# Villen-Lab/pyAscore

Measured on AMD Instinct MI355X. Metric: PSMs/sec (Ascore.score) at 1/2/4/8 MI355X + HBM-roofline %, higher is better.
Workload: dtype f32/f64 scalar + i32 counts

## Files before the change

pyascore_amd/csrc/fused_core.hip.h:

```cpp
#ifndef PYA_FUSED_CORE_H
#define PYA_FUSED_CORE_H
#include "score_core.hip.h"
#include "localize_core.hip.h"

#define FUSED_ROUND 3

struct FusedLds {
    uint16_t *grid;
    uint4 *cum_lut;
    PeakEntry *peaks;
    float2 *resd;
    uint8_t *rkl;
    uint32_t *rec;
    float *wsl;
    float *mass_l;
    uint32_t *flag_l;
    uint8_t *site_pos;
    float *selm;
    unsigned char *sort_raw;
    PushedEntry *pushed;
    unsigned long long *site_alt;
    uint32_t *site_max, *site_tie, *n_pushed;
    float *sc;
    uint32_t *c_tr, *c_cnt;
    uint32_t *bad_tasks;
    uint32_t *t_lo, *t_off;
    float *srt_v;
    uint8_t *srt_h;
    int32_t *c_depth;
    uint32_t *c_site;
};

__host__ __device__ static inline size_t fused_align16(size_t v) { return (v + 15) & ~(size_t)15; }
__host__ __device__ static inline size_t fused_sort_bytes(uint32_t n) {
    if (n <= 64) return ((size_t)n * 10 + 15) & ~(size_t)15;
    return (((size_t)n * 6 + 15) & ~(size_t)15) + ((size_t)n / 64 + 2) * 16 + 2 * 128 * 2;
}
__host__ __device__ static inline uint32_t fused_site_cap(uint32_t push_cap) {
    const uint32_t v = (push_cap + 3u) & ~3u;
    return v > 64u ? 64u : (v < 4u ? 4u : v);
}
__host__ __device__ static inline size_t fused_post_bytes(uint32_t n_cap, uint32_t push_cap, uint32_t ent_cap, uint32_t ndir,
                                                          bool multi_z) {
    return fused_align16(fused_sort_bytes(n_cap)) + (size_t)push_cap * 16 + (size_t)fused_site_cap(push_cap) * 16 + 16 +
           (size_t)(1 + FUSED_ROUND) * 40 + (size_t)FUSED_ROUND * (16 * ndir + 4 + 4) + 16 + 64 +
           (multi_z ? fused_align16((size_t)FUSED_ROUND * ndir * 2 * ent_cap * 4) +
                          fused_align16((size_t)FUSED_ROUND * ndir * 2 * ent_cap)
                    : 0);
}
__host__ __device__ static inline size_t fused_walk_bytes(uint32_t cap) {
    return 16 * 16 + ((size_t)cap + PYA_TABLE_PAD) * 8;
}
__host__ __device__ static inline size_t fused_kept_bytes(uint32_t n_cap, uint32_t stride, uint32_t pos_cap, uint32_t ent_cap,
                                                          uint32_t ndir) {
    return fused_align16(((size_t)pos_cap + 1) * 8) + fused_align16((size_t)ent_cap * stride) + (size_t)n_cap * 16 + 256 +
           fused_align16((size_t)pos_cap + 1) + (size_t)(1 + FUSED_ROUND) * ndir * ent_cap * 4;
}
__host__ __device__ static inline size_t fused_lds_bytes(uint32_t cap, uint32_t n_cap, uint32_t stride, uint32_t pos_cap,
                                                         uint32_t ent_cap, uint32_t push_cap, uint32_t ndir, bool multi_z) {
    const size_t walk = fused_walk_bytes(cap), post = fused_post_bytes(n_cap, push_cap, ent_cap, ndir, multi_z);
    return PYA_GRID_CELLS * 2 + fused_align16(walk > post ? walk : post) +
           fused_kept_bytes(n_cap, stride, pos_cap, ent_cap, ndir) + 16;
}

DEV FusedLds fused_carve(unsigned char *raw, uint32_t cap, uint32_t n_cap, uint32_t stride, uint32_t pos_cap,
                         uint32_t ent_cap, uint32_t push_cap, uint32_t ndir, bool multi_z) {
    FusedLds f;
    f.grid = (uint16_t *)raw;
    size_t o = PYA_GRID_CELLS * 2;
    f.cum_lut = (uint4 *)(raw + o);
    f.peaks = (PeakEntry *)(raw + o + 16 * 16);
    f.sort_raw = raw + o;
    size_t q = o + fused_align16(fused_sort_bytes(n_cap));
    f.pushed = (PushedEntry *)(raw + q);
    q += (size_t)push_cap * sizeof(PushedEntry);
    const size_t sc = fused_site_cap(push_cap);
    f.site_alt = (unsigned long long *)(raw + q);
    q += sc * 8;
    f.site_max = (uint32_t *)(raw + q);
    q += sc * 4;
    f.site_tie = (uint32_t *)(raw + q);
    q += sc * 4;
    f.n_pushed = (uint32_t *)(raw + q);
    q += 16;
    f.sc = (float *)(raw + q);
    q += (size_t)(1 + FUSED_ROUND) * 40;
    f.c_tr = (uint32_t *)(raw + q);
    q += (size_t)FUSED_ROUND * ndir * 8;
    f.c_cnt = (uint32_t *)(raw + q);
    q += (size_t)FUSED_ROUND * ndir * 8;
    f.c_depth = (int32_t *)(raw + q);
    q += FUSED_ROUND * 4;
    f.c_site = (uint32_t *)(raw + q);
    q += FUSED_ROUND * 4;
    f.bad_tasks = (uint32_t *)(raw + q);
    q += 16;
    f.t_lo = (uint32_t *)(raw + q);
    f.t_off = f.t_lo + 8;
    q += 64;
    f.srt_v = (float *)(raw + q);
    q += fused_align16((size_t)FUSED_ROUND * ndir * 2 * ent_cap * 4);
    f.srt_h = (uint8_t *)(raw + q);
    const size_t walk = fused_walk_bytes(cap), post = fused_post_bytes(n_cap, push_cap, ent_cap, ndir, multi_z);
    o += fused_align16(walk > post ? walk : post);
    f.resd = (float2 *)(raw + o);
    o += fused_align16(((size_t)pos_cap + 1) * 8);
    f.rkl = (uint8_t *)(raw + o);
    o += fused_align16((size_t)ent_cap * stride);
    f.rec = (uint32_t *)(raw + o);
    o += (size_t)n_cap * 12;
    f.wsl = (float *)(raw + o);
    o += (size_t)n_cap * 4;
    f.mass_l = (float *)(raw + o);
    f.flag_l = (uint32_t *)(raw + o + 128);
    f.site_pos = (uint8_t *)(raw + o + 256);
    f.selm = (float *)(raw + o + 256 + fused_align16((size_t)pos_cap + 1));
    return f;
}


template <bool BZ>
DEV void walk_record_steps(const float2 *&rp, int rstride, StepBits &bits, float &running, const uint4 *lut, CumCounts &cum,
                           const PeakTable &tab, int zmax, double A, double B, uint8_t *&ro, int stride, int count) {
    for (int i = 0; i < count; i++, rp += rstride) {
        const float2 mm = *rp;
        running = (bits.next() ? mm.y : mm.x) + running;
        const double m = BZ ? (double)running + A : ((double)running + A) - B;
        for (int z = 1; z <= zmax; z++, ro += stride) {
            const Look k = look4(tab, charge_mz(m, z));
            int rk = k.best;
            if (k.more()) rk = look_rest(tab, k);
            cum.add(lut[rk]);
            *ro = (uint8_t)rk;
        }
    }
}
DEV CumCounts walk_record(const float2 *resd, const uint4 *lut, const PeakTable &tab, int L, int zmax, uint64_t resmask, int dir,
                          double A, double B, bool all_b_zero, uint8_t *rkl, int stride, int w) {
    const uint64_t tmask = dir ? (__brevll(resmask) >> (64 - L)) : resmask;
    const float2 *rp = resd + (dir ? L - 1 : 0);
    const int rstride = dir ? -1 : 1;
    uint8_t *ro = rkl + w;
    float running = 0.f;
    CumCounts cum = {0u, 0u, 0u};
    if (tab.half_check) {
        const uint32_t tlo = (uint32_t)tmask, thi = (uint32_t)(tmask >> 32);
        for (int step = 0; step + 1 < L; step++, rp += rstride) {
            const float2 mm = *rp;
            const uint32_t word = step < 32 ? tlo : thi;
            const bool mod = (word >> (step & 31)) & 1u;
            running = (mod ? mm.y : mm.x) + running;
            const double m = ((double)running + A) - B;
            for (int z = 1; z <= zmax; z++, ro += stride) {
                const int rk = match_rank_lds(tab, charge_mz(m, z));
                cum.add(lut[rk]);
                *ro = (uint8_t)rk;
            }
        }
        return cum;
    }
    const uint64_t M = msb_first_from(tmask, 0);
    const int n = L - 1;
    for (int seg = 0; seg < 2; seg++) {
        StepBits bits = {seg ? (uint32_t)M : (uint32_t)(M >> 32)};
        int c = (n < seg * 32 + 32 ? n : seg * 32 + 32) - seg * 32;
        if (c < 0) c = 0;
        if (all_b_zero) walk_record_steps<true>(rp, rstride, bits, running, lut, cum, tab, zmax, A, B, ro, stride, c);
        else walk_record_steps<false>(rp, rstride, bits, running, lut, cum, tab, zmax, A, B, ro, stride, c);
    }
    return cum;
}

DEV void walk_mz_only(const float2 *resd, int L, int zmax, uint64_t resmask, int dir, double A, double B, float *out) {
    const uint64_t tmask = dir ? (__brevll(resmask) >> (64 - L)) : resmask;
    const uint64_t M = msb_first_from(tmask, 0);
    const float2 *rp = resd + (dir ? L - 1 : 0);
    const int rstride = dir ? -1 : 1;
    const int Lm1 = L - 1;
    float running = 0.f;
    int step = 0;
    for (int seg = 0; seg < 2; seg++) {
        StepBits bits = {seg ? (uint32_t)M : (uint32_t)(M >> 32)};
        const int end = Lm1 < seg * 32 + 32 ? Lm1 : seg * 32 + 32;
        for (; step < end; step++, rp += rstride) {
            const float2 mm = *rp;
            running = (bits.next() ? mm.y : mm.x) + running;
            const double m = ((double)running + A) - B;
            out[step] = (float)(m + 1.007825);
            for (int z = 2; z <= zmax; z++) out[(z - 1) * Lm1 + step] = charge_mz(m, z);
        }
    }
}

DEV void walk_sums_only(const float2 *resd, int L, uint64_t resmask, int dir, float *out) {
    const uint64_t tmask = dir ? (__brevll(resmask) >> (64 - L)) : resmask;
    const uint64_t M = msb_first_from(tmask, 0);
    const float2 *rp = resd + (dir ? L - 1 : 0);
    const int rstride = dir ? -1 : 1;
    const int Lm1 = L - 1;
    float running = 0.f;
    int step = 0;
    for (int seg = 0; seg < 2; seg++) {
        StepBits bits = {seg ? (uint32_t)M : (uint32_t)(M >> 32)};
        const int end = Lm1 < seg * 32 + 32 ? Lm1 : seg * 32 + 32;
        for (; step < end; step++, rp += rstride) {
            const float2 mm = *rp;
            running = (bits.next() ? mm.y : mm.x) + running;
            out[step] = running;
        }
    }
}

DEV int partners_in_run(const float *run, int n, int p2, float me, int side, float err) {
    int j = 0;
    for (int step = p2 >> 1; step > 0; step >>= 1) {
        const int probe = j + step;
        const float o = probe - 1 < n ? run[probe - 1] : __builtin_huge_valf();
        const float dd = side ? (o - me) : (me - o);
        if (side ? (dd <= -err) : (dd >= err)) j = probe;
    }
    int cnt = 0;
    for (int q = j; q < j + 2 && q < n; q++) {
        const float dd = side ? (run[q] - me) : (me - run[q]);
        cnt += (__builtin_fabsf(dd) < err) ? 1 : 0;
    }
    return cnt;
}

#define FUSED_LOCAL_CHUNKS 8
struct LocalTable {
    const float *mz;
    const uint8_t *rank;
    int R, status;
};

template <bool BOTH, bool ZM, bool WIDE = false>
DEV bool fused_body(const BatchDev &b, uint32_t psm, unsigned char *lds_raw, uint32_t cap, uint32_t n_cap, uint32_t stride,
                    uint32_t pos_cap, uint32_t ent_cap, uint32_t push_cap, const LocalTable *local = nullptr) {
    const int lane = lane_id();
    const DevConfig *cfg = b.cfg;
    const int ndir = BOTH ? 2 : 1;
    const FusedLds f = fused_carve(lds_raw, cap, n_cap, stride, pos_cap, ent_cap, push_cap, (uint32_t)ndir, ZM);
    STAMP_BEGIN();
    STAMP_T(b, 38, false);
    float lmz[FUSED_LOCAL_CHUNKS];
    uint32_t lrk[FUSED_LOCAL_CHUNKS];
    if (local) {
#pragma unroll
        for (int q = 0; q < FUSED_LOCAL_CHUNKS; q++) {
            const int i = q * 64 + lane_id();
            lmz[q] = i < local->R ? local->mz[i] : __builtin_huge_valf();
            lrk[q] = i < local->R ? (uint32_t)local->rank[i] : (uint32_t)PYA_NO_MATCH;
        }
        wave_lds_sync();
    }
    if (lane < 32) {
        f.mass_l[lane] = cfg->res_mass[lane];
        f.flag_l[lane] = cfg->res_modifiable[lane];
    }
    const uint64_t *dw = b.desc + (size_t)psm * PYA_DESC_WORDS;
    const int64_t p0 = (int64_t)dw[0], pep0 = (int64_t)dw[1], s0 = (int64_t)dw[2], a0 = (int64_t)dw[3];
    const uint64_t w4 = dw[4], w5 = dw[5];
    const int L = (int)(w4 & 0xffffu), n_aux = (int)((w4 >> 16) & 0xffffu), k = (int)((w4 >> 32) & 0xffffu);
    const int zmax = ZM ? (int)(w4 >> 56) : 1;
    const int N = (int)(uint32_t)w5;
    const uint64_t *order = b.order_tab + (uint32_t)(w5 >> 32);
    const int status = local ? local->status : b.status[psm];
    const int R = local ? local->R : (int)b.ret_n[psm];

    const uint32_t max_k = b.max_k;
    float *out_asc = b.ascores + (size_t)psm * max_k;
    uint64_t *out_alt = b.alt_mask + (size_t)psm * max_k;
    for (uint32_t a = lane; a < max_k; a += 64) {
        out_asc[a] = 0.f;
        out_alt[a] = 0ull;
    }
    if (status != PYA_ST_OK) {
        if (lane == 0) {
            b.best_score[psm] = -1.f;
            b.best_sig[psm] = 0ull;
            b.n_sig_out[psm] = -1;
        }
        return false;
    }
    STAMP_T(b, 39, false);
    const bool two_pass = BOTH && WIDE && N > 32;
    const int s = (BOTH && !two_pass) ? (lane & 31) : lane;
    const int dir = BOTH ? (two_pass ? 0 : (lane >> 5)) : (cfg->n_fwd > 0 ? 0 : 1);
    const bool active = s < N;
    const uint32_t letter = lane < L ? (uint32_t)b.pep[pep0 + lane] : (uint32_t)'A';
    const uint64_t bits = active ? order[s] : 0ull;
    uint32_t aux_pos = 0;
    float aux_mass = 0.f;
    if (lane < n_aux) {
        aux_pos = b.aux_pos[a0 + lane];
        aux_mass = b.aux_mass[a0 + lane];
    }
    if (local) {
#pragma unroll
        for (int q = 0; q < FUSED_LOCAL_CHUNKS; q++) {
            const int i = q * 64 + lane;
            if (i < R + PYA_TABLE_PAD) {
                PeakEntry e;
                e.mz = lmz[q];
                e.rank = lrk[q];
                f.peaks[i] = e;
            }
        }
    } else {
        copy_peak_table(b.ret + p0, R, f.peaks, lane, 64);
    }
    PeakTable tab;
    tab.e = f.peaks;
    tab.g_cell = nullptr;
    tab.g_e = b.ret + p0;
    tab.n = R;
    tab.err = cfg->mz_error;
    tab.half_check = cfg->mz_error > 0.49f;
    double Af = 0., Bf = 0., Ab = 0., Bb = 0.;
    if (cfg->n_fwd > 0) type_constants(cfg->types[0], &Af, &Bf);
    if (cfg->n_fwd < cfg->n_types) type_constants(cfg->types[cfg->n_fwd], &Ab, &Bb);
    wave_lds_sync();
    STAMP_T(b, 48, false);
    float m0, m1;
    uint64_t site_mask;
    {
        const bool in = lane < L;
        const uint32_t li = (letter - 'A') & 31u;
        m0 = f.mass_l[li];
        const bool modifiable = in && ((f.flag_l[li] & 1u) || (cfg->allow_n && lane == 0) || (cfg->allow_c && lane == L - 1));
        m1 = m0 + cfg->mod_mass;
        for (int base = 0; base < n_aux; base += 64) {
            const int n = n_aux - base < 64 ? n_aux - base : 64;
            if (base > 0) {
                aux_pos = 0;
                aux_mass = 0.f;
                if (lane < n) {
                    aux_pos = b.aux_pos[a0 + base + lane];
                    aux_mass = b.aux_mass[a0 + base + lane];
                }
            }
            for (int j = 0; j < n; j++) {
                const uint32_t pos = (uint32_t)__builtin_amdgcn_readlane((int)aux_pos, j);
                const float am = __int_as_float(__builtin_amdgcn_readlane(__float_as_int(aux_mass), j));
                const int idx = pos > 0 ? (int)pos - 1 : 0;
                if (idx == lane) {
                    m0 += am;
                    m1 += am;
                }
            }
        }
        site_mask = __ballot(modifiable);
        if (in) f.resd[lane] = make_float2(m0, m1);
        if (modifiable) f.site_pos[mask_rank(site_mask)] = (uint8_t)lane;
    }
    STAMP_T(b, 49, false);
    grid_build(&tab, f.grid);
    STAMP_T(b, 50, false);
    if (lane < 16) f.cum_lut[lane] = fused_cum_entry((uint32_t)lane);
    const int Lm1 = L - 1;
    const uint64_t resmask = deposit_sites(bits, site_mask);
    const int w = !active ? (int)stride - 1 : (BOTH ? dir * N + s : s);
    const bool presorted = !__any(lane < L && !(m0 > 0.f && m1 > 0.f));
    const float wide_min = 2.f * cfg->mz_error + 0.02f;
    const bool wide = !__any(lane < L && !(m0 > wide_min && m1 > wide_min));
    wave_lds_sync();
    STAMP_T(b, 40, false);
    CumCounts cum = walk_record(f.resd, f.cum_lut, tab, L, zmax, resmask, dir, dir ? Ab : Af, dir ? Bb : Bf, Bf == 0. && Bb == 0.,
                                f.rkl, (int)stride, w);
    if (two_pass) {
        const CumCounts back = walk_record(f.resd, f.cum_lut, tab, L, zmax, resmask, 1, Ab, Bb, Bf == 0. && Bb == 0., f.rkl, (int)stride,
                                           active ? N + s : (int)stride - 1);
        cum.a += back.a;
        cum.b += back.b;
        cum.c += back.c;
    } else if (BOTH) {
        uint32_t *r3 = f.rec + (size_t)s * 3;
        if (active && lane >= 32) {
            r3[0] = cum.a;
            r3[1] = cum.b;
            r3[2] = cum.c;
        }
        wave_lds_sync();
        if (active && lane < 32) {
            cum.a += r3[0];
            cum.b += r3[1];
            cum.c += r3[2];
        }
    }
    wave_lds_sync();
    STAMP_T(b, 41, false);

    const uint32_t nfrag = (uint32_t)ndir * (uint32_t)Lm1 * (uint32_t)zmax;
    int fail = 0;
    float ws = 0.f;
    if (active && (!BOTH || two_pass || lane < 32)) {
        ws = -1.f;
        if (nfrag <= b.lut_n_max) {
            double sum = 0.;
#pragma unroll
            for (int d = 0; d < PYA_NTOP; d++) {
                const float sc = lut_score(b, (uint32_t)d, cum.at(d), nfrag);
                const float prod = cfg->weights[d] * sc;
                sum = sum + (double)prod;
            }
            ws = (float)sum;
        } else {
            fail = 1;
        }
        uint32_t *r3 = f.rec + (size_t)s * 3;
        r3[0] = cum.a;
        r3[1] = cum.b;
        r3[2] = cum.c;
        f.wsl[s] = ws;
    }
    if (__any(fail)) {
        if (lane == 0) {
            b.status[psm] = PYA_ST_LUT_RANGE;
            b.best_score[psm] = -1.f;
            b.best_sig[psm] = 0ull;
            b.n_sig_out[psm] = -1;
        }
        return false;
    }
    wave_lds_sync();
    STAMP_T(b, 42, false);

    bool declined = !presorted || (b.debug & 512);
    const bool sig_lane = lane < N;
    const uint64_t my_bits = bits;
    const float my_ws = sig_lane ? f.wsl[lane] : 0.f;
    float best_ws = 0.f;
    uint64_t best_bits = 0ull;
    uint32_t best_i = 0, np = 0;
    if (!declined) {
        const uint32_t u = sig_lane ? __float_as_uint(my_ws) : 0u;
        const uint32_t kmax = wave_max_u32(u);
        const uint64_t at_max = __ballot(sig_lane && u == kmax);
        best_i = (uint32_t)__builtin_ctzll(at_max);
        if (lane == 0) *f.n_pushed = 0;
        if ((uint32_t)lane < fused_site_cap(push_cap)) {
            f.site_max[lane] = 0;
            f.site_tie[lane] = 0;
            f.site_alt[lane] = 0ull;
        }
        if (__popcll(at_max) != 1 || (b.debug & 1024)) {
            const SortLds srt = sort_carve(f.sort_raw, N);
            if (sig_lane) {
                srt.key[lane] = my_ws;
                srt.idx[lane] = (uint16_t)lane;
            }
            wave_lds_sync();
            if (!(b.debug & 8) && sort_introsort_loop<true, true>(srt, N, true)) declined = true;
            const uint64_t m2 = __ballot(sig_lane && __float_as_uint(srt.key[lane]) == kmax);
            best_i = srt.idx[__builtin_ctzll(m2)];
        }
        best_ws = __uint_as_float(kmax);
        best_bits = __shfl(my_bits, (int)best_i, 64);
        wave_lds_sync();
    }
    STAMP_T(b, 43, false);
    if (!declined) {
        const uint64_t gone = best_bits & ~my_bits, came = my_bits & ~best_bits;
        const bool single = sig_lane && __popcll(gone) == 1 && __popcll(came) == 1;
        const int a = single ? __popcll(best_bits & (gone - 1)) : 0;
        const uint32_t u = __float_as_uint(my_ws);
        if (single) atomicMax(&f.site_max[a], u);
        wave_lds_sync();
        if (single && u == f.site_max[a]) {
            if ((double)__builtin_fabsf(best_ws - my_ws) < 1e-6) {
                f.site_tie[a] = 1u;
                atomicOr(&f.site_alt[a], 1ull << f.site_pos[__builtin_ctzll(came)]);
            } else {
                const uint32_t slot = atomicAdd(f.n_pushed, 1u);
                if (slot < push_cap) {
                    PushedEntry pe;
                    pe.bits = my_bits;
                    pe.ws = my_ws;
                    pe.idx = (uint32_t)lane;
                    f.pushed[slot] = pe;
                }
            }
        }
        wave_lds_sync();
        np = *f.n_pushed;
        if (np > push_cap) np = push_cap;
        if (b.debug & 16) np = 0;
    }
    STAMP_T(b, 44, false);
    float my_asc = __builtin_huge_valf();
    const float err = cfg->mz_error;
    const FastDiv divL = fastdiv_make((uint32_t)(Lm1 > 0 ? Lm1 : 1));
    int p2 = 1;
    while (p2 <= Lm1) p2 <<= 1;
    for (uint32_t e0 = 0; !declined && e0 < np; e0 += FUSED_ROUND) {
        const int nc = (int)(np - e0) < FUSED_ROUND ? (int)(np - e0) : FUSED_ROUND;
        const int S = 1 + nc;
        if (lane < S * ndir && (e0 == 0 || lane >= ndir)) {
            const int sg = lane / ndir, d = lane - sg * ndir;
            const uint64_t sb = sg == 0 ? best_bits : f.pushed[e0 + sg - 1].bits;
            const int dd = BOTH ? d : (cfg->n_fwd > 0 ? 0 : 1);
            if (ZM) walk_mz_only(f.resd, L, zmax, deposit_sites(sb, site_mask), dd, dd ? Ab : Af, dd ? Bb : Bf,
                                 f.selm + (size_t)lane * ent_cap);
            else walk_sums_only(f.resd, L, deposit_sites(sb, site_mask), dd, f.selm + (size_t)lane * ent_cap);
        }
        if (!ZM) {
            wave_lds_sync();
            const int l0 = e0 == 0 ? 0 : ndir, nl = S * ndir - l0;
            for (int i = lane; i < nl * Lm1; i += 64) {
                const int lq = (int)fastdiv((uint32_t)i, divL), st = i - lq * Lm1;
                const int dd = BOTH ? ((l0 + lq) & 1) : (cfg->n_fwd > 0 ? 0 : 1);
                float *at = f.selm + (size_t)(l0 + lq) * ent_cap + st;
                const double m = ((double)*at + (dd ? Ab : Af)) - (dd ? Bb : Bf);
                *at = (float)(m + 1.007825);
            }
        }
        for (int i = (e0 == 0 ? 0 : 10) + lane; i < S * 10; i += 64) {
            const int sg = i / 10, d = i - sg * 10;
            const uint32_t who = sg == 0 ? best_i : f.pushed[e0 + sg - 1].idx;
            const uint32_t cum = (f.rec[(size_t)who * 3 + (d >> 2)] >> ((d & 3) * 8)) & 0xffu;
            f.sc[i] = b.lut[lut_row(nfrag) + (uint32_t)d * (nfrag + 1) + cum];
        }
        wave_lds_sync();
        if (lane < nc) {
            const PushedEntry pe = f.pushed[e0 + lane];
            const uint64_t gone = best_bits & ~pe.bits, came = pe.bits & ~best_bits;
            const int a = __popcll(best_bits & (gone - 1));
            atomicOr(&f.site_alt[a], 1ull << f.site_pos[__builtin_ctzll(came)]);
            f.c_site[lane] = (uint32_t)a;
        }
        {
            const int c = lane >> 4, d = lane & 15;
            const bool on = c < nc && d < PYA_NTOP;
            uint32_t key = 0;
            if (on) {
                const float diff = f.sc[d] - f.sc[(c + 1) * 10 + d];
                key = diff > 0.f ? __float_as_uint(diff) : 0u;
            }
            if (lane < nc) f.c_depth[lane] = 0;
            wave_lds_sync();
            if (on && key) atomicMax((uint32_t *)&f.c_depth[c], key);
            wave_lds_sync();
            const uint64_t at_max = __ballot(on && key && key == (uint32_t)f.c_depth[c]);
            wave_lds_sync();
            if (lane < nc) {
                const uint32_t m16 = (uint32_t)(at_max >> (16 * lane)) & 0xffffu;
                f.c_depth[lane] = m16 ? __builtin_ctz(m16) : 0;
            }
        }
        if (lane < nc * ndir * 2) {
            f.c_tr[lane] = 0;
            f.c_cnt[lane] = 0;
        }
        if (lane == 0) *f.bad_tasks = 0u;
        wave_lds_sync();
        STAMP_T(b, 45, false);
        const int ents = Lm1 * zmax;
        const int items_all = nc * ndir * 2 * ents;
        const FastDiv divE = fastdiv_make((uint32_t)(ents > 0 ? ents : 1));
        const bool spans = !ZM && wide && !(b.debug & 2048);
        const bool zm_clusters = ZM && !(b.debug & 2048);
        int items = items_all;
        if (spans) {
            const int ntask = nc * ndir;
            if (lane < ntask) {
                const int c = lane / ndir, d = lane - c * ndir;
                const int dd = BOTH ? d : (cfg->n_fwd > 0 ? 0 : 1);
                const uint64_t diff = best_bits ^ f.pushed[e0 + c].bits;
                const int r_lo = (int)f.site_pos[__builtin_ctzll(diff)];
                const int r_hi = (int)f.site_pos[63 - __builtin_clzll(diff)];
                const int lo = dd ? L - 1 - r_hi : r_lo, hi = dd ? L - 1 - r_lo : r_hi;
                f.t_lo[lane] = (uint32_t)lo;
                f.t_off[lane] = (uint32_t)(2 * (hi - lo));
            }
            wave_lds_sync();
            uint32_t acc = 0;
            for (int t = 0; t < ntask; t++) {
                const uint32_t n = f.t_off[t];
                wave_lds_sync();
                if (lane == 0) f.t_off[t] = acc;
                acc += n;
            }
            if (lane == 0) f.t_off[ntask] = acc;
            items = (int)acc;
            wave_lds_sync();
        }
        if (!(b.debug & 1) && !zm_clusters)
        for (int base = 0; base < items; base += 64) {
            const int e = base + lane;
            if (e < items) {
                int task, side, en;
                if (spans) {
                    const int ntask = nc * ndir;
                    task = 0;
                    for (int t = 1; t < ntask; t++) task += (uint32_t)e >= f.t_off[t] ? 1 : 0;
                    const int rem = e - (int)f.t_off[task];
                    const int len = (int)(f.t_off[task + 1] - f.t_off[task]) >> 1;
                    side = rem >= len ? 1 : 0;
                    en = (int)f.t_lo[task] + rem - side * len;
                } else {
                    const uint32_t ts = fastdiv((uint32_t)e, divE);
                    en = e - (int)ts * ents;
                    side = (int)ts & 1;
                    task = (int)ts >> 1;
                }
                const int z0 = zmax == 1 ? 0 : (int)fastdiv((uint32_t)en, divL), i = en - z0 * Lm1;
                const int d = BOTH ? task & 1 : 0;
                const int c = BOTH ? task >> 1 : task;
                const float *la = f.selm + (size_t)d * ent_cap;
                const float *lb = f.selm + (size_t)((1 + c) * ndir + d) * ent_cap;
                const float *mine = side ? lb : la, *others = side ? la : lb;
                const float me = mine[en];
                int total = 0;
                {
                    const float *other = others + z0 * Lm1;
                    float df[4];
                    bool ok[4], sk[4];
#pragma unroll
                    for (int uu = 0; uu < 4; uu++) {
                        const int q = i - 1 + uu;
                        ok[uu] = q >= 0 && q < Lm1;
                        const float o = ok[uu] ? other[q] : (q < 0 ? -__builtin_huge_valf() : __builtin_huge_valf());
                        df[uu] = me - o;
                        sk[uu] = df[uu] >= err;
                    }
                    const int w1 = (ok[1] && __builtin_fabsf(df[1]) < err) ? 1 : 0;
                    const int w2 = (ok[2] && __builtin_fabsf(df[2]) < err) ? 1 : 0;
                    const int w3 = (ok[3] && __builtin_fabsf(df[3]) < err) ? 1 : 0;
                    int cnt = -1;
                    if (sk[0] && !sk[1]) cnt = w1 + w2;
                    else if (sk[1] && !sk[2]) cnt = w2 + w3;
                    if (cnt < 0) cnt = partners_in_run(other, Lm1, p2, me, side, err);
                    total = cnt;
                }
                for (int zz = 0; zz < zmax; zz++)
                    if (zz != z0) total += partners_in_run(others + zz * Lm1, Lm1, p2, me, side, err);
                if (total > 1 || (b.debug & 2048)) {
                    atomicOr(f.bad_tasks, 1u << task);
                } else if (total == 0) {
                    const uint32_t who = side ? f.pushed[e0 + c].idx : best_i;
                    atomicAdd(&f.c_tr[task * 2 + side], 1u);
                    if ((int)f.rkl[(size_t)(i * zmax + z0) * stride + (d * N + (int)who)] <= f.c_depth[c])
                        atomicAdd(&f.c_cnt[task * 2 + side], 1u);
                }
            }
        }
        wave_lds_sync();
        const uint32_t bad = zm_clusters ? (1u << (nc * ndir)) - 1u : *f.bad_tasks;
        if (!ZM && bad) declined = true;
        if (ZM && bad && !(b.debug & 1)) {
            for (int base = 0; base < items_all; base += 64) {
                const int e = base + lane;
                if (e < items_all) {
                    const uint32_t ts = fastdiv((uint32_t)e, divE);
                    const int en = e - (int)ts * ents;
                    const int z0 = zmax == 1 ? 0 : (int)fastdiv((uint32_t)en, divL), i = en - z0 * Lm1;
                    const int side = (int)ts & 1;
                    const int d = BOTH ? ((int)ts >> 1) & 1 : 0;
                    const int c = BOTH ? (int)ts >> 2 : (int)ts >> 1;
                    const int task = c * ndir + d;
                    if ((bad >> task) & 1u) {
                        const float *mine = f.selm + (size_t)((side ? (1 + c) * ndir : 0) + d) * ent_cap;
                        const float me = mine[en];
                        int pos = i;
                        for (int zz = 0; zz < zmax; zz++) {
                            if (zz == z0) continue;
                            const float *run = mine + zz * Lm1;
                            int j = 0;
                            for (int step = p2 >> 1; step > 0; step >>= 1) {
                                const int probe = j + step;
                                if (probe - 1 < Lm1 && (zz < z0 ? run[probe - 1] <= me : run[probe - 1] < me)) j = probe;
                            }
                            pos += j;
                        }
                        const uint32_t who = side ? f.pushed[e0 + c].idx : best_i;
                        const size_t at = (size_t)(task * 2 + side) * ent_cap + pos;
                        f.srt_v[at] = me;
                        f.srt_h[at] = (int)f.rkl[(size_t)(i * zmax + z0) * stride + (d * N + (int)who)] <= f.c_depth[c] ? 1 : 0;
                    }
                }
            }
            wave_lds_sync();
            if (zm_clusters) {
                int p2e = 1;
                while (p2e <= ents) p2e <<= 1;
                for (int base = 0; base < items_all; base += 64) {
                    const int e = base + lane;
                    if (e >= items_all) continue;
                    const uint32_t ts = fastdiv((uint32_t)e, divE);
                    const int i = e - (int)ts * ents;
                    const int side = (int)ts & 1;
                    const int d = BOTH ? ((int)ts >> 1) & 1 : 0;
                    const int c = BOTH ? (int)ts >> 2 : (int)ts >> 1;
                    const int task = c * ndir + d;
                    const float *va = f.srt_v + (size_t)(task * 2) * ent_cap, *vb = va + ent_cap;
                    const uint8_t *ha = f.srt_h + (size_t)(task * 2) * ent_cap, *hb = ha + ent_cap;
                    const float *mine = side ? vb : va, *other = side ? va : vb;
                    const float me = mine[i];
                    int j = 0;
                    for (int step = p2e >> 1; step > 0; step >>= 1) {
                        const int probe = j + step;
                        if (probe - 1 < ents && (side ? other[probe - 1] <= me : other[probe - 1] < me)) j = probe;
                    }
                    const float before_own = i > 0 ? mine[i - 1] : -__builtin_huge_valf();
                    const float before_other = j > 0 ? other[j - 1] : -__builtin_huge_valf();
                    if (!(me - before_own >= err && me - before_other >= err)) continue;
                    int ia = side ? j : i, ib = side ? i : j;
                    uint32_t tr0 = 0, tr1 = 0, n0 = 0, n1 = 0;
                    float reached = -__builtin_huge_valf();
                    for (bool first = true;; first = false) {
                        const float xa = ia < ents ? va[ia] : __builtin_huge_valf();
                        const float xb = ib < ents ? vb[ib] : __builtin_huge_valf();
                        const float next = xa <= xb ? xa : xb;
                        if (next == __builtin_huge_valf()) break;
                        if (!first && next - reached >= err) break;
                        if (__builtin_fabsf(xa - xb) < err) {
                            ia++;
                            ib++;
                            reached = __builtin_fmaxf(reached, xa > xb ? xa : xb);
                        } else if (xa < xb) {
                            tr0++;
                            n0 += ha[ia++];
                            reached = __builtin_fmaxf(reached, xa);
                        } else {
                            tr1++;
                            n1 += hb[ib++];
                            reached = __builtin_fmaxf(reached, xb);
                        }
                    }
                    if (tr0) atomicAdd(&f.c_tr[task * 2], tr0);
                    if (tr1) atomicAdd(&f.c_tr[task * 2 + 1], tr1);
                    if (n0) atomicAdd(&f.c_cnt[task * 2], n0);
                    if (n1) atomicAdd(&f.c_cnt[task * 2 + 1], n1);
                }
            } else
            if (lane < nc * ndir && ((bad >> lane) & 1u)) {
                const float *va = f.srt_v + (size_t)(lane * 2) * ent_cap, *vb = va + ent_cap;
                const uint8_t *ha = f.srt_h + (size_t)(lane * 2) * ent_cap, *hb = ha + ent_cap;
                uint32_t tr0 = 0, tr1 = 0, n0 = 0, n1 = 0;
                int ia = 0, ib = 0;
                while (ia < ents || ib < ents) {
                    if (ib == ents) {
                        tr0++;
                        n0 += ha[ia++];
                    } else if (ia == ents) {
                        tr1++;
                        n1 += hb[ib++];
                    } else {
                        const float xa = va[ia], xb = vb[ib];
                        if (__builtin_fabsf(xa - xb) < err) {
                            ia++;
                            ib++;
                        } else if (xa < xb) {
                            tr0++;
                            n0 += ha[ia++];
                        } else {
                            tr1++;
                            n1 += hb[ib++];
                        }
                    }
                }
                f.c_tr[lane * 2] = tr0;
                f.c_tr[lane * 2 + 1] = tr1;
                f.c_cnt[lane * 2] = n0;
                f.c_cnt[lane * 2 + 1] = n1;
            }
            wave_lds_sync();
        }
        STAMP_T(b, 46, false);
        if (!declined) {
            float asc_l = 0.f;
            if (lane < nc) {
                uint32_t tr0 = 0, tr1 = 0, n0 = 0, n1 = 0;
                for (int d = 0; d < ndir; d++) {
                    const int t = lane * ndir + d;
                    tr0 += f.c_tr[t * 2];
                    tr1 += f.c_tr[t * 2 + 1];
                    n0 += f.c_cnt[t * 2];
                    n1 += f.c_cnt[t * 2 + 1];
                }
                const uint32_t depth = (uint32_t)f.c_depth[lane];
                if (tr0 > b.lut_n_max || tr1 > b.lut_n_max) {
                    fail = 1;
                } else {
                    const float sc0 = b.lut[lut_row(tr0) + depth * (tr0 + 1) + n0];
                    const float sc1 = b.lut[lut_row(tr1) + depth * (tr1 + 1) + n1];
                    asc_l = sc0 - sc1;
                }
            }
            for (int c = 0; c < nc; c++) {
                const float asc = __shfl(asc_l, c, 64);
                if (lane == (int)f.c_site[c]) my_asc = asc < my_asc ? asc : my_asc;
            }
        }
        wave_lds_sync();
    }
    if (declined) {
        if (sig_lane) {
            b.ws[s0 + lane] = my_ws;
            if (b.rec) {
                const uint32_t *r3 = f.rec + (size_t)lane * 3;
                uint32_t *dst = b.rec + (s0 + lane) * PYA_REC_WORDS;
                uint32_t cum[PYA_NTOP];
#pragma unroll
                for (int d = 0; d < PYA_NTOP; d++) cum[d] = (r3[d >> 2] >> ((d & 3) * 8)) & 0xffu;
#pragma unroll
                for (int d = 0; d < PYA_NTOP; d += 2) dst[d >> 1] = cum[d] | (cum[d + 1] << 16);
                dst[5] = nfrag;
            }
        }
        ((uint64_t *)(b.grid + (size_t)psm * PYA_GRID_CELLS))[lane] = ((const uint64_t *)f.grid)[lane];
        if (lane == 0) b.ws_top[(size_t)psm * 4 + 1] = 0u;
        return true;
    }
    STAMP_T(b, 47, false);
    if (lane < k && f.site_tie[lane]) my_asc = 0.f < my_asc ? 0.f : my_asc;
    if (lane < k && lane < (int)max_k) {
        out_asc[lane] = my_asc;
        out_alt[lane] = f.site_alt[lane];
    }
    const bool any_fail = __any(fail != 0);
    if (lane == 0) {
        b.best_score[psm] = best_ws;
        b.best_sig[psm] = best_bits;
        b.n_sig_out[psm] = N;
        if (any_fail) b.status[psm] = PYA_ST_LUT_RANGE;
    }
    return false;
}

#endif
```

pyascore_amd/csrc/host_one.cpp:

```cpp
#include "host_internal.h"
#include <climits>

namespace {
const size_t kOneFlag = 0, kOneStatus = 64, kOneBest = 128, kOneAsc = 192, kOneAlt = 448, kOneMz = 1024,
             kOneInt = kOneMz + (size_t)PYA_FAST_PEAKS * 8, kOneBytes = kOneInt + (size_t)PYA_FAST_PEAKS * 8;

int one_prepare(pya_handle *h, uint32_t n_sig) {
    pya_handle::One &o = h->one;
    if (!o.host) {
        HIPCHK(h, hipHostMalloc((void **)&o.host, kOneBytes, hipHostMallocMapped | hipHostMallocCoherent));
        HIPCHK(h, hipHostGetDevicePointer((void **)&o.host_dev, o.host, 0));
        std::memset(o.host, 0, 1024);
        HIPCHK(h, hipStreamCreateWithFlags(&o.stream, hipStreamNonBlocking));
    }
    if (!o.ws.p || o.sig_cap < n_sig) {
        const uint32_t cap = std::max<uint32_t>(1024, next_pow2(n_sig));
        const size_t bytes = 4096 + ((size_t)PYA_FAST_PEAKS + 8) * sizeof(PeakEntry) + PYA_GRID_CELLS * 2 + 4096 +
                             (size_t)cap * (4 + PYA_REC_WORDS * 4 + 4) + 1024;
        HIPCHK(h, hipStreamSynchronize(o.stream));
        if (o.view && h->kept == o.view) h->kept = nullptr;
        o.last_keep = false;
        HIPCHK(h, o.ws.alloc(bytes));
        if (h->kn.slow_null_stream) {
            if (!o.probe.p) HIPCHK(h, o.probe.alloc((size_t)256 << 20));
            HIPCHK(h, hipMemset(o.probe.p, 0, (size_t)256 << 20));
        }
        HIPCHK(h, hipMemsetAsync(o.ws.p, 0, bytes, o.stream));
        HIPCHK(h, hipStreamSynchronize(o.stream));
        o.sig_cap = cap;
        unsigned char *w = o.ws.p;
        BatchDev &d = o.dev;
        std::memset(&d, 0, sizeof d);
        size_t at = 0;
        auto take = [&](size_t n) { unsigned char *q = w + at; at += (n + 255) & ~(size_t)255; return q; };
        d.peak_off = (const int64_t *)take(16);
        d.pep_off = (const int64_t *)take(16);
        d.aux_off = (const int64_t *)take(16);
        d.sig_off = (const int64_t *)take(16);
        d.ret_off = (const int64_t *)take(16);
        d.pep = (const uint8_t *)take(PYA_MAX_L);
        d.n_of_mod = (const int32_t *)take(4);
        d.max_charge = (const int32_t *)take(4);
        d.aux_pos = (const uint32_t *)take(PYA_ONE_MAX_AUX * 4);
        d.aux_mass = (const float *)take(PYA_ONE_MAX_AUX * 4);
        d.n_sites = (const uint8_t *)take(4);
        d.n_sig = (const uint32_t *)take(4);
        d.order_off = (const uint32_t *)take(4);
        d.desc = (const uint64_t *)take(PYA_DESC_WORDS * 8);
        d.status = (int32_t *)take(4);
        d.ret_n = (uint32_t *)take(4);
        d.ws_top = (uint32_t *)take(16);
        uint32_t *redo = (uint32_t *)take(4 * 80);
        d.redo_count = redo;
        d.redo_ids = redo + 64;
        d.redo3_count = redo + 66;
        d.redo3_ids = redo + 70;
        d.redo3b_count = redo + 67;
        d.redo3b_ids = redo + 72;
        d.redo4_count = redo + 68;
        d.redo4_ids = redo + 74;
        d.grid = (uint16_t *)take(PYA_GRID_CELLS * 2);
        d.ret = (PeakEntry *)take(((size_t)PYA_FAST_PEAKS + 8) * sizeof(PeakEntry));
        d.ws = (float *)take((size_t)cap * 4);
        d.rec = (uint32_t *)take((size_t)cap * PYA_REC_WORDS * 4);
        d.sorted_idx = (uint32_t *)take((size_t)cap * 4);
        d.mz = (const double *)(o.host_dev + kOneMz);
        d.inten = (const double *)(o.host_dev + kOneInt);
        d.best_score = (float *)(o.host_dev + kOneBest);
        d.n_sig_out = (int32_t *)(o.host_dev + kOneBest + 8);
        d.best_sig = (uint64_t *)(o.host_dev + kOneBest + 16);
        d.ascores = (float *)(o.host_dev + kOneAsc);
        d.alt_mask = (uint64_t *)(o.host_dev + kOneAlt);
    }
    return PYA_OK;
}

int one_run(pya_handle *h, bool keep, uint32_t max_k) {
    pya_handle::One &o = h->one;
    const OneMeta &m = o.meta;
    BatchDev d = o.dev;
    shared_tables(h, d);
    d.max_k = max_k;
    d.keep = keep ? 1u : 0u;
    d.debug = h->kn.debug & 0xffffu;
    const uint32_t L = m.L, z = (uint32_t)m.max_charge, k = (uint32_t)m.n_of_mod, ns = m.n_sites, N = m.n_sig;
    Bucket bk;
    bk.take_knobs(h->kn);
    bk.cover(*h, N, L, z, k, ns, (L - 1) * z * (uint32_t)h->cfg.n_uniq);
    const uint32_t cap = (m.n_peaks + 31u) & ~31u;
    const uint32_t prefix = score_prefix(h, N), compact = score_compact(h->cfg, z);
    const bool both = h->cfg.n_fwd > 0 && h->cfg.n_fwd < h->cfg.n_types;
    uint32_t use_fused = 0, f_n_cap = 4, f_stride = 8, f_ent = 1, f_push = 8;
    const uint32_t frags = (both ? 2u : 1u) * (L - 1) * z;
    if (!keep && plain_types(h->cfg) && !h->kn.no_fused && k < ns && N > 0 && N <= (both ? 32u : 64u) && frags <= 255u) {
        use_fused = both ? 1u : 2u;
        f_n_cap = (N + 3u) & ~3u;
        f_stride = (both ? 2u : 1u) * f_n_cap + 4u;
        f_ent = std::max<uint32_t>((L - 1) * z, 1);
        f_push = std::max<uint32_t>(8u, bk.push_cap());
    }
    if (pya_one_lds_bytes(cap, prefix, with_nl(h->cfg), compact, bk.push_cap(), bk.n_cap, bk.pos_cap, bk.pool_cap(), bk.sb(), use_fused,
                          f_n_cap, f_stride, f_ent, f_push, z > 1) > kMaxLds)
        return PYA_ERR_STATE;
    volatile uint32_t *flag = (volatile uint32_t *)(o.host + kOneFlag);
    volatile int32_t *echo = (volatile int32_t *)(o.host + kOneStatus + 4);
    volatile int32_t *n_sig_word = (volatile int32_t *)(o.host + kOneBest + 8);
    const int32_t kUnset = INT32_MIN;
    *n_sig_word = kUnset;
    const auto t_launch = std::chrono::steady_clock::now();
    int e = pya_launch_one(&d, &m, cap, prefix, with_nl(h->cfg), compact, bk.push_cap(), bk.n_cap, bk.pos_cap, bk.pool_cap(),
                           bk.sb(), bk.gtp(), use_fused, f_n_cap, f_stride, f_ent, f_push, z > 1 ? 1u : 0u,
                           (int32_t *)(o.host_dev + kOneStatus), (uint32_t *)(o.host_dev + kOneFlag), o.stream);
    if (e) return h->hip_fail((hipError_t)e, "score (one PSM) launch");
    const auto t0 = std::chrono::steady_clock::now();
    o.t_sum[2] += std::chrono::duration<double>(t0 - t_launch).count();
    auto published = [&]() { return *flag == m.seq && (uint32_t)*echo == m.seq && *n_sig_word != kUnset; };
    for (uint64_t spins = 0; !published(); spins++) {
        __builtin_ia32_pause();
        if ((spins & 0xffff) == 0xffff && std::chrono::steady_clock::now() - t0 > std::chrono::seconds(2)) {
            HIPCHK(h, hipStreamSynchronize(o.stream));
            if (!published()) return h->fail(PYA_ERR_HIP, 0, "the kernel finished without publishing its results");
        }
    }
    std::atomic_thread_fence(std::memory_order_acquire);
    o.t_sum[3] += std::chrono::duration<double>(std::chrono::steady_clock::now() - t0).count();
    o.last_keep = keep;
    o.last_max_k = max_k;
    if (keep) {
        if (!o.view) o.view = new pya_plan;
        pya_plan *p = o.view;
        p->h = h;
        p->settings_gen = h->settings_gen;
        p->flags = PYA_FLAG_KEEP;
        p->n_psm = 1;
        p->peak_cap = cap;
        p->max_k = max_k;
        p->sig_off = {0, (int64_t)N};
        p->pep_off = {0, (int64_t)L};
        p->n_sig = {N};
        p->order_off = {m.order_off};
        p->max_charge = {m.max_charge};
        p->d_rec.adopt(d.rec, (size_t)N * PYA_REC_WORDS);
        p->d_sorted.adopt(d.sorted_idx, N);
        p->d_ws.adopt(d.ws, N);
        p->dev = d;
        p->quiesced = true;
        p->ran = true;
        p->last_stream = o.stream;
        if (h->kept && h->kept != p) pya_plan_destroy(h->kept);
        h->kept = p;
    } else if (h->kept && h->kept == o.view) {
        h->kept = nullptr;
    }
    return PYA_OK;
}
}

extern "C" int pya_score_one(pya_handle *h, const double *mz, const double *inten, uint64_t n_peaks, const uint8_t *pep,
                             uint64_t L, int32_t n_of_mod, int32_t max_charge, const uint32_t *aux_pos, const float *aux_mass,
                             uint64_t n_aux, uint32_t flags, const pya_results *out) {
    if (!h || !out) return PYA_ERR_ARG;
    const auto t_in = std::chrono::steady_clock::now();
    h->err.clear();
    h->err_index = -1;
    h->last_status.clear();
    h->evid_valid = false;
    h->ions_valid = false;
    h->sites_valid = false;
    h->probs_valid = false;
    h->ranked_valid = false;
    h->rollup_valid = false;
    h->mzp_valid = false;
    h->quant_valid = false;
    h->pform_valid = false;
    h->pfq_valid = false;
    h->cov_valid = false;
    if (flags & PYA_FLAG_COVERAGE)
        return h->fail(PYA_ERR_ARG, -1, "pya_score_one does not take PYA_FLAG_COVERAGE: score the PSM as a batch of one (pya_score_batch)");
    if (flags & PYA_FLAG_EVIDENCE)
        return h->fail(PYA_ERR_ARG, -1, "pya_score_one does not take PYA_FLAG_EVIDENCE: score the PSM as a batch of one (pya_score_batch)");
    if (flags & PYA_FLAG_IONS)
        return h->fail(PYA_ERR_ARG, -1, "pya_score_one does not take PYA_FLAG_IONS: score the PSM as a batch of one (pya_score_batch)");
    if (flags & PYA_FLAG_SITES)
        return h->fail(PYA_ERR_ARG, -1, "pya_score_one does not take PYA_FLAG_SITES: score the PSM as a batch of one (pya_score_batch)");
    if (flags & PYA_FLAG_PROBS)
        return h->fail(PYA_ERR_ARG, -1, "pya_score_one does not take PYA_FLAG_PROBS: score the PSM as a batch of one (pya_score_batch)");
    if (flags & PYA_FLAG_RANKED)
        return h->fail(PYA_ERR_ARG, -1, "pya_score_one does not take PYA_FLAG_RANKED: score the PSM as a batch of one (pya_score_batch)");
    if (flags & PYA_FLAG_PEPTIDOFORMS)
        return h->fail(PYA_ERR_ARG, -1, "pya_score_one does not take PYA_FLAG_PEPTIDOFORMS: score the PSM as a batch of one (pya_score_batch)");
    if (flags & PYA_FLAG_QUANT)
        return h->fail(PYA_ERR_ARG, -1, "pya_score_one does not take PYA_FLAG_QUANT: score the PSM as a batch of one (pya_score_batch)");
    if (flags & PYA_FLAG_PFORM_QUANT)
        return h->fail(PYA_ERR_ARG, -1, "pya_score_one does not take PYA_FLAG_PFORM_QUANT: score the PSM as a batch of one (pya_score_batch)");
    if (flags & PYA_FLAG_MZ_PROFILE)
        return h->fail(PYA_ERR_ARG, -1, "pya_score_one does not take PYA_FLAG_MZ_PROFILE: score the PSM as a batch of one (pya_score_batch)");
    if (flags & PYA_FLAG_RECALIBRATE)
        return h->fail(PYA_ERR_ARG, -1, "pya_score_one does not take PYA_FLAG_RECALIBRATE: score the PSM as a batch of one (pya_score_batch)");
    if (flags & PYA_FLAG_ROLLUP)
        return h->fail(PYA_ERR_ARG, -1, "pya_score_one does not take PYA_FLAG_ROLLUP: score the PSM as a batch of one (pya_score_batch)");
    if (h->kn.no_tiny) return PYA_ERR_STATE;
    if (!mz || !inten || !pep) return h->fail(PYA_ERR_ARG, -1, "NULL array");
    if (!out->best_score || !out->best_sig || !out->n_sig || !out->ascores || !out->alt_mask)
        return h->fail(PYA_ERR_ARG, -1, "NULL array in results");
    if (n_aux && (!aux_pos || !aux_mass)) return h->fail(PYA_ERR_ARG, -1, "NULL fixed-modification arrays");
    char msg[kPsmMsg];
    uint32_t ns = 0, per_type = 0;
    uint64_t N = 0;
    int code = check_psm_shape(h, 0, (int64_t)n_peaks, (int64_t)L, n_of_mod, max_charge, pep, aux_pos, (int64_t)n_aux, &ns, msg);
    if (!code) code = check_psm_limits(h, 0, (int64_t)L, n_of_mod, max_charge, ns, &N, &per_type, msg);
    if (code) return h->fail(code, 0, "%s", msg);
    if (h->all_general() || n_peaks > PYA_FAST_PEAKS || L > PYA_FAST_PEPTIDE_LEN || N > PYA_FAST_SIGNATURES || per_type > PYA_FAST_FRAGMENTS_PER_TYPE) return PYA_ERR_STATE;
    if (n_aux > PYA_ONE_MAX_AUX || (uint32_t)n_of_mod > 64u) return PYA_ERR_STATE;
    if (out->max_k < (uint32_t)std::max(n_of_mod, 1)) return h->fail(PYA_ERR_ARG, -1, "results.max_k is smaller than n_of_mod");
    HIPCHK(h, hipSetDevice(h->device));
    int rc = sync_config(h);
    if (rc) return rc;
    uint32_t ooff = 0;
    if (N) {
        uint32_t &co = h->shape_cache[ns][n_of_mod];
        if (co == 0xffffffffu) co = shape_offset(h, ns, (uint32_t)n_of_mod);
        ooff = co;
    }
    rc = ensure_lut(h, per_type * (uint32_t)h->cfg.n_types);
    if (rc) return rc;
    rc = upload_shared_tables(h);
    if (rc) return rc;
    rc = one_prepare(h, (uint32_t)N);
    if (rc) return rc;
    pya_handle::One &o = h->one;
    const auto t_copy = std::chrono::steady_clock::now();
    std::memcpy(o.host + kOneMz, mz, (size_t)n_peaks * 8);
    std::memcpy(o.host + kOneInt, inten, (size_t)n_peaks * 8);
    OneMeta &m = o.meta;
    std::memset(&m, 0, sizeof m);
    std::memcpy(m.pep, pep, (size_t)L);
    m.n_peaks = (uint32_t)n_peaks;
    m.L = (uint32_t)L;
    m.n_aux = (uint32_t)n_aux;
    m.n_sig = (uint32_t)N;
    m.order_off = ooff;
    m.seq = ++o.seq ? o.seq : ++o.seq;
    m.n_of_mod = n_of_mod;
    m.max_charge = max_charge;
    m.n_sites = ns;
    for (uint64_t a = 0; a < n_aux; a++) {
        m.aux_pos[a] = aux_pos[a];
        m.aux_mass[a] = aux_mass[a];
    }
    pack_desc_tail(L, n_aux, n_of_mod, ns, max_charge, (uint32_t)N, ooff, m.desc);
    o.have_last = true;
    const uint32_t mk = out->max_k;
    if (mk > 64) return PYA_ERR_STATE;
    const auto t_run = std::chrono::steady_clock::now();
    o.t_sum[0] += std::chrono::duration<double>(t_copy - t_in).count();
    o.t_sum[1] += std::chrono::duration<double>(t_run - t_copy).count();
    rc = one_run(h, (flags & PYA_FLAG_KEEP) != 0, mk);
    if (rc) return rc;
    const auto t_out = std::chrono::steady_clock::now();
    const int32_t st = *(const int32_t *)(o.host + kOneStatus);
    rc = check_status(h, &st, 1, false);
    if (rc) return rc;
    out->best_score[0] = *(const float *)(o.host + kOneBest);
    out->n_sig[0] = *(const int32_t *)(o.host + kOneBest + 8);
    out->best_sig[0] = *(const uint64_t *)(o.host + kOneBest + 16);
    std::memcpy(out->ascores, o.host + kOneAsc, (size_t)mk * 4);
    std::memcpy(out->alt_mask, o.host + kOneAlt, (size_t)mk * 8);
    o.t_sum[4] += std::chrono::duration<double>(std::chrono::steady_clock::now() - t_out).count();
    for (int i = 0; i < 4; i++) o.t_dev[i] += 1e-8 * (double)*(const int32_t *)(o.host + kOneStatus + 8 + 4 * i);
    o.t_cycles += (double)*(const int32_t *)(o.host + kOneStatus + 24);
    o.t_calls++;
    return PYA_OK;
}

extern "C" int pya_one_times(pya_handle *h, double us[12]) {
    if (!h || !us) return PYA_ERR_ARG;
    pya_handle::One &o = h->one;
    for (int i = 0; i < 12; i++) us[i] = 0.;
    for (int i = 0; i < 5; i++) {
        us[i] = o.t_calls ? 1e6 * o.t_sum[i] / (double)o.t_calls : 0.;
        o.t_sum[i] = 0.;
    }
    for (int i = 0; i < 4; i++) {
        us[6 + i] = o.t_calls ? 1e6 * o.t_dev[i] / (double)o.t_calls : 0.;
        o.t_dev[i] = 0.;
    }
    us[5] = (double)o.t_calls;
    us[10] = o.t_calls ? o.t_cycles / (double)o.t_calls : 0.;
    o.t_cycles = 0.;
    o.t_calls = 0;
    return PYA_OK;
}

extern "C" int pya_rescore_last_keep(pya_handle *h) {
    if (!h) return PYA_ERR_ARG;
    if (!h->one.have_last) return h->fail(PYA_ERR_STATE, -1, "no PSM scored with pya_score_one yet");
    if (h->one.last_keep && h->kept == h->one.view) return PYA_OK;
    HIPCHK(h, hipSetDevice(h->device));
    h->one.meta.seq = ++h->one.seq ? h->one.seq : ++h->one.seq;
    return one_run(h, true, h->one.last_max_k);
}
```

Before: 205.9 million.

## Split fused fragment walk across idle helper lanes in both-direction mode

Measured after the change: 214.7 million, median of 6. +4.2%, better.

```diff
diff --git a/pyascore_amd/csrc/fused_core.hip.h b/pyascore_amd/csrc/fused_core.hip.h
--- a/pyascore_amd/csrc/fused_core.hip.h
+++ b/pyascore_amd/csrc/fused_core.hip.h
@@ -171,6 +171,79 @@
     return cum;
 }
 
+template <bool BZ>
+DEV void walk_record_pairs(const float2 *&rp, int rstride, StepBits &bits, float &running, const uint4 *lut, CumCounts &cum,
+                           const PeakTable &tab, double A, double B, uint8_t *&ro, int stride, int count) {
+    int i = 0;
+    for (; i + 2 <= count; i += 2, rp += 2 * rstride, ro += 2 * stride) {
+        const float2 ma = rp[0], mb = rp[rstride];
+        const float ra = (bits.next() ? ma.y : ma.x) + running;
+        const float rb = (bits.next() ? mb.y : mb.x) + ra;
+        running = rb;
+        const double da = BZ ? (double)ra + A : ((double)ra + A) - B, db = BZ ? (double)rb + A : ((double)rb + A) - B;
+        const Look ka = look4(tab, charge_mz(da, 1)), kb = look4(tab, charge_mz(db, 1));
+        int rka = ka.best, rkb = kb.best;
+        if (ka.more()) rka = look_rest(tab, ka);
+        if (kb.more()) rkb = look_rest(tab, kb);
+        cum.add(lut[rka]);
+        cum.add(lut[rkb]);
+        ro[0] = (uint8_t)rka;
+        ro[stride] = (uint8_t)rkb;
+    }
+    if (i < count) walk_record_steps<BZ>(rp, rstride, bits, running, lut, cum, tab, 1, A, B, ro, stride, 1);
+}
+
+template <bool BZ>
+DEV CumCounts walk_record_split(const float2 *resd, const uint4 *lut, const PeakTable &tab, int L, int x, uint64_t resmask, int dir,
+                                bool helper, double Af, double Bf, double Ab, double Bb, uint8_t *rkl, int stride, int w, int N) {
+    const int n = L - 1;
+    const uint64_t fwd_m = __brevll(resmask), back_m = resmask << (64 - L);
+    uint64_t M = dir ? back_m : fwd_m;
+    const float2 *rp = resd + (dir ? n : 0);
+    int rstride = dir ? -1 : 1;
+    double A = dir ? Ab : Af, B = dir ? Bb : Bf;
+    float running = 0.f;
+    if (!helper) {
+        StepBits pre = {(uint32_t)(M >> 32)};
+        int i = 0;
+        for (; i + 4 <= x; i += 4, rp += 4 * rstride) {
+            const float2 m0 = rp[0], m1 = rp[rstride], m2 = rp[2 * rstride], m3 = rp[3 * rstride];
+            running = (pre.next() ? m0.y : m0.x) + running;
+            running = (pre.next() ? m1.y : m1.x) + running;
+            running = (pre.next() ? m2.y : m2.x) + running;
+            running = (pre.next() ? m3.y : m3.x) + running;
+        }
+        for (; i < x; i++, rp += rstride) {
+            const float2 mm = *rp;
+            running = (pre.next() ? mm.y : mm.x) + running;
+        }
+        M <<= x;
+    }
+    StepBits bits = {(uint32_t)(M >> 32)};
+    uint8_t *ro = rkl + (helper ? 0 : x * stride) + w;
+    CumCounts cum = {0u, 0u, 0u};
+    walk_record_pairs<BZ>(rp, rstride, bits, running, lut, cum, tab, A, B, ro, stride, x);
+    if (helper) {
+        rp = resd + n;
+        rstride = -1;
+        bits.w = (uint32_t)(back_m >> 32);
+        running = 0.f;
+        A = Ab;
+        B = Bb;
+        ro = rkl + N + w;
+    }
+    const int T = n - x;
+    for (int done = x; done < T;) {
+        if (done == 32 && !helper) bits.w = (uint32_t)M;
+        int next = done < 2 * x ? 2 * x : T;
+        if (done < 32 && next > 32) next = 32;
+        if (!(helper && done >= 2 * x))
+            walk_record_pairs<BZ>(rp, rstride, bits, running, lut, cum, tab, A, B, ro, stride, next - done);
+        done = next;
+    }
+    return cum;
+}
+
 DEV void walk_mz_only(const float2 *resd, int L, int zmax, uint64_t resmask, int dir, double A, double B, float *out) {
     const uint64_t tmask = dir ? (__brevll(resmask) >> (64 - L)) : resmask;
     const uint64_t M = msb_first_from(tmask, 0);
@@ -288,8 +361,11 @@
     const int s = (BOTH && !two_pass) ? (lane & 31) : lane;
     const int dir = BOTH ? (two_pass ? 0 : (lane >> 5)) : (cfg->n_fwd > 0 ? 0 : 1);
     const bool active = s < N;
+    const bool split = BOTH && !ZM && !WIDE && 3 * N <= 64 && L - 1 >= 6 && !(cfg->mz_error > 0.49f) && !(b.debug & 0x08000000u);
+    const int hs = lane - (lane < 32 ? N : 2 * N);
+    const bool helper = split && !active && hs < N;
     const uint32_t letter = lane < L ? (uint32_t)b.pep[pep0 + lane] : (uint32_t)'A';
-    const uint64_t bits = active ? order[s] : 0ull;
+    const uint64_t bits = active ? order[s] : (helper ? order[hs] : 0ull);
     uint32_t aux_pos = 0;
     float aux_mass = 0.f;
     if (lane < n_aux) {
@@ -366,8 +442,23 @@
     const bool wide = !__any(lane < L && !(m0 > wide_min && m1 > wide_min));
     wave_lds_sync();
     STAMP_T(b, 40, false);
-    CumCounts cum = walk_record(f.resd, f.cum_lut, tab, L, zmax, resmask, dir, dir ? Ab : Af, dir ? Bb : Bf, Bf == 0. && Bb == 0.,
-                                f.rkl, (int)stride, w);
+    CumCounts cum;
+    if (split) {
+        const int sd = helper ? 0 : dir, sw = helper ? hs : w, x = Lm1 / 3;
+        cum = (Bf == 0. && Bb == 0.)
+                  ? walk_record_split<true>(f.resd, f.cum_lut, tab, L, x, resmask, sd, helper, Af, Bf, Ab, Bb, f.rkl, (int)stride, sw, N)
+                  : walk_record_split<false>(f.resd, f.cum_lut, tab, L, x, resmask, sd, helper, Af, Bf, Ab, Bb, f.rkl, (int)stride, sw, N);
+        const int from = s + N < 32 ? s + N : s + 2 * N;
+        const uint32_t ha = __shfl(cum.a, from, 64), hb = __shfl(cum.b, from, 64), hc = __shfl(cum.c, from, 64);
+        if (active && lane < 32) {
+            cum.a += ha;
+            cum.b += hb;
+            cum.c += hc;
+        }
+    } else {
+        cum = walk_record(f.resd, f.cum_lut, tab, L, zmax, resmask, dir, dir ? Ab : Af, dir ? Bb : Bf, Bf == 0. && Bb == 0., f.rkl,
+                          (int)stride, w);
+    }
     if (two_pass) {
         const CumCounts back = walk_record(f.resd, f.cum_lut, tab, L, zmax, resmask, 1, Ab, Bb, Bf == 0. && Bb == 0., f.rkl, (int)stride,
                                            active ? N + s : (int)stride - 1);
diff --git a/pyascore_amd/csrc/host_one.cpp b/pyascore_amd/csrc/host_one.cpp
--- a/pyascore_amd/csrc/host_one.cpp
+++ b/pyascore_amd/csrc/host_one.cpp
@@ -82,7 +82,7 @@
     shared_tables(h, d);
     d.max_k = max_k;
     d.keep = keep ? 1u : 0u;
-    d.debug = h->kn.debug & 0xffffu;
+    d.debug = h->kn.debug & (0xffffu | 0x08000000u);
     const uint32_t L = m.L, z = (uint32_t)m.max_charge, k = (uint32_t)m.n_of_mod, ns = m.n_sites, N = m.n_sig;
     Bucket bk;
     bk.take_knobs(h->kn);
```
